# mmorise/World

Hardware: AMD Instinct MI355X
Metric: analysis frames/sec (Harvest+CheapTrick+D4C, 48 kHz, 5 ms hop) (higher is better)
Workload: dtype f64; 1 GPU; configs[1]: 1 x (48 kHz, 10 s) utterance(s) per step, Harvest+CheapTrick+D4C, fft_size=2048, frame_period=5 ms, inputs/outputs in HBM, 12 independent jobs in flight (one HIP stream + context each, a different utterance per job); utterances_per_gpu=1, jobs_in_flight=12, parallelism=single GPU, no collective

## Files before the change

world_amd/csrc/bandfilter.h:

```cpp
#pragma once
#include "trace.h"
#include "common.h"

namespace world_hip {

constexpr int kBpThreads = 256;
constexpr int kOutPer = 8;
constexpr int kTile = kBpThreads * kOutPer;
constexpr int kSegTiles = 2;
constexpr int kSeg = kTile * kSegTiles;
constexpr int kSegCap = kSeg / 2 + 2;

__host__ __device__ __forceinline__ int pad8(int i) { return i + (i >> 3); }

struct BandJob {
  const double *in;
  int in_len;
  int n;
  const double *taps;
  int ntap;
  int shift;
  int max_ntap;
  int nseg;
  double *seg_events;
// ... 147 lines not shown
    const int kbase = sub + tid * PER;
    unsigned mask[4] = {0u, 0u, 0u, 0u};
    {
      double a = kbase < len + 2 ? sample(kbase) : 0.0, b = kbase + 1 < len + 2 ? sample(kbase + 1) : 0.0;
#pragma unroll
      for (int q = 0; q < PER; ++q) {
        const double c = kbase + q + 2 < len + 2 ? sample(kbase + q + 2) : 0.0;
        const int i = t0 + kbase + q;
        const bool live = kbase + q < len;
        const double da = b - a, db = c - b;
        const bool r01 = live && i <= n - 2, r23 = live && i <= n - 3;
        if (r01 && 0.0 < a && b <= 0.0) mask[0] |= 1u << q;
        if (r01 && a < 0.0 && 0.0 <= b) mask[1] |= 1u << q;
        if (r23 && 0.0 < da && db <= 0.0) mask[2] |= 1u << q;
        if (r23 && da < 0.0 && 0.0 <= db) mask[3] |= 1u << q;
        a = b; b = c;
      }
    }
    WH_ACC_END(0);
    WH_ACC_BEGIN;
    unsigned long long packed = 0;
#pragma unroll
    for (int fam = 0; fam < 4; ++fam) packed |= (unsigned long long)__builtin_popcount(mask[fam]) << (16 * fam);
    unsigned long long total, off = block_excl_scan_u64<PRE>(packed, &total, scratch);
    WH_ACC_END(1);
    WH_ACC_BEGIN;
    int at[4];
#pragma unroll
    for (int fam = 0; fam < 4; ++fam) at[fam] = count[fam] + (int)((off >> (16 * fam)) & 0xFFFF);
    while ((mask[0] | mask[1] | mask[2] | mask[3]) != 0u) {
#pragma unroll
      for (int fam = 0; fam < 4; ++fam) {
        if (mask[fam] != 0u) {
          const int q = __builtin_ctz(mask[fam]);
          mask[fam] &= mask[fam] - 1;
          double a = sample(kbase + q), b = sample(kbase + q + 1);
          if (fam >= 2) { const double c = sample(kbase + q + 2); a = b - a; b = c - b; }
          if (at[fam] < cap) ev[fam * fam_stride + at[fam]] = fine_edge_fast(t0 + kbase + q + 1, a, b);
          ++at[fam];
        }
      }
    }
#pragma unroll
    for (int fam = 0; fam < 4; ++fam) count[fam] += (int)((total >> (16 * fam)) & 0xFFFF);
    WH_ACC_END(2);
  }
  WH_ACC_FLUSH(32, tid == 0);
}

__device__ __forceinline__ void band_events_segment(const BandJob &job, int seg) {
  DYN_LDS(lds);
  const int tid = threadIdx.x, nt = blockDim.x;
  const int n = job.n;
  const int seg_begin = seg * kSeg;
  int *cnt_out = job.seg_count + seg;
  if (seg_begin >= n) {
    if (tid == 0) for (int fam = 0; fam < 4; ++fam) cnt_out[(size_t)fam * job.nseg] = 0;
    return;
  }
  const int seg_end = imin(n, seg_begin + kSeg);
  const bool trace_me = blockIdx.x == 5 && blockIdx.y == 20; (void)trace_me;
  WH_ACC_DECL;
  WH_ACC_BEGIN;
  double *taps = reinterpret_cast<double *>(lds);
  double *yt = taps + (job.max_ntap + 1);
  double *s = yt + pad8(kTile + 2 + job.max_ntap + 3 + 8) + 1;
  double *scratch = s + pad8(kTile + 4) + 1;
  for (int j = tid; j < job.ntap; j += nt) taps[j] = job.taps[j];

  double *ev = job.seg_events + (size_t)seg * kSegCap;
  const size_t fam_stride = (size_t)job.nseg * kSegCap;
  int count[4] = {0, 0, 0, 0};
  const bool pipelined = tile_fits_regs(job);
  TileRegs pre;
  if (pipelined) tile_fetch(job, seg_begin, pre);
  WH_ACC_END(0);
  for (int t0 = seg_begin; t0 < seg_end; t0 += kTile) {
    WH_ACC_BEGIN;
    if (pipelined) {
      __syncthreads();
      tile_commit(job, pre, yt);
      __syncthreads();
      if (t0 + kTile < seg_end) tile_fetch(job, t0 + kTile, pre);
      WH_ACC_END(1);
      WH_ACC_BEGIN;
      fir_compute(job, taps, yt, s);
    } else {
      fir_tile(job, taps, t0, yt, s);
    }
    if (job.quirk) {
      const double qc = job.quirk[0], qs = job.quirk[1], q0 = job.quirk[2], w = job.quirk[3];
      const int n0 = t0 + tid + job.quirk_delay;
      double sn, cs, sr, cr;
      sincospi(n0 * w, &sn, &cs);
      sincospi(nt * w, &sr, &cr);
      const double sign = (n0 & 1) ? -1.0 : 1.0;
      for (int k = tid, j = 0; k < kTile + 2; k += nt, ++j) {
        const double flip = ((nt & 1) && (j & 1)) ? -sign : sign;
        s[pad8(k)] += flip * (qc * cs + qs * sn + q0);
        const double c2 = cs * cr - sn * sr;
        sn = sn * cr + cs * sr;
        cs = c2;
      }
      __syncthreads();
    }
    WH_ACC_END(2);
    WH_ACC_BEGIN;
    tile_events([&](int k) { return s[pad8(k)]; }, t0, kTile, n, ev, fam_stride, count, kSegCap, scratch);
    WH_ACC_END(3);
  }
  WH_ACC_SET(4, job.ntap);
  WH_ACC_FLUSH(16, tid == 0);
  if (tid == 0)
    for (int fam = 0; fam < 4; ++fam) cnt_out[(size_t)fam * job.nseg] = imin(count[fam], kSegCap);
}

inline size_t compact_lds_bytes(int nseg) { return 64 * sizeof(double) + sizeof(int) * (size_t)(nseg + 1); }
__device__ __forceinline__ void compact_event_segments(const double *seg_events, const int *seg_count, int nseg, int seg_cap,
                                                       double *events, int ev_cap, int *ev_count, char *lds) {
  double *scratch = reinterpret_cast<double *>(lds);
  int *pre = reinterpret_cast<int *>(scratch + 64);
  const int tid = threadIdx.x, nt = blockDim.x;
  int running = 0;
  for (int s0 = 0; s0 < nseg; s0 += nt) {
    const int s = s0 + tid;
    const int c = s < nseg ? seg_count[s] : 0;
    int tot;
    const int at = block_excl_scan_int(c, &tot, scratch);
    if (s < nseg) pre[s] = running + at;
    running += tot;
  }
  if (tid == 0) pre[nseg] = running;
  __syncthreads();
  const int total = imin(running, ev_cap);
  constexpr int kB = 8;
  int s = 0;
  for (int j0 = tid; j0 < total; j0 += kB * nt) {
    double v[kB];
#pragma unroll
    for (int q = 0; q < kB; ++q) {
      const int j = imin(j0 + q * nt, total - 1);
      while (j >= pre[s + 1]) ++s;
      v[q] = seg_events[(size_t)s * seg_cap + (j - pre[s])];
    }
#pragma unroll
    for (int q = 0; q < kB; ++q) if (j0 + q * nt < total) events[j0 + q * nt] = v[q];
  }
  if (tid == 0) *ev_count = total;
}

__device__ __forceinline__ double interval_loc(const double *e, int k, double fs) { return (e[k] + e[k + 1]) / 2.0 / fs; }
__device__ __forceinline__ double interval_f0(const double *e, int k, double fs) { return fs / (e[k + 1] - e[k]); }

__device__ __forceinline__ int intervals_at_or_before(const double *e, int n_int, double fs, double t) {
  int lo = 0, hi = n_int;
  if (n_int > 8) {
    const double first = interval_loc(e, 0, fs), last = interval_loc(e, n_int - 1, fs);
    const double r = (t - first) / (last - first) * (n_int - 1);
    int g = r < 0.0 ? 0 : (r > n_int - 1.0 ? n_int - 1 : static_cast<int>(r));
    if (interval_loc(e, g, fs) <= t) {
      lo = g + 1;
      for (int step = 1, q = g + 1; ; q += step, step <<= 1) {
        if (q >= n_int) break;
        if (interval_loc(e, q, fs) > t) { hi = q; break; }
        lo = q + 1;
      }
    } else {
      hi = g;
      for (int step = 1, q = g - 1; ; q -= step, step <<= 1) {
        if (q < 0) break;
        if (interval_loc(e, q, fs) <= t) { lo = q + 1; break; }
        hi = q;
      }
    }
  }
  while (lo < hi) {
    int mid = (lo + hi) >> 1;
    if (interval_loc(e, mid, fs) <= t) lo = mid + 1; else hi = mid;
  }
  return lo;
}

__device__ __forceinline__ int intervals_at_or_before_group(const double *e, int n_int, double fs, double t, int group, int sub) {
#ifdef WORLD_EMU
  (void)group; (void)sub;
  return intervals_at_or_before(e, n_int, fs, t);
#else
  if (n_int <= 0) return 0;
  const double first = interval_loc(e, 0, fs), last = interval_loc(e, n_int - 1, fs);
  if (!(first <= t)) return 0;
  if (last <= t) return n_int;
  int lo = 0, hi = n_int - 1;
  auto ones_at = [&](int idx, bool valid) {
    const bool pred = valid && interval_loc(e, idx, fs) <= t;
    return __popc((unsigned)(__ballot(pred) >> (32 * group)));
  };
  if (hi - lo > 32) {
    const double r = (t - first) / (last - first) * (n_int - 1);
    const int g = r < 0.0 ? 0 : (r > n_int - 1.0 ? n_int - 1 : static_cast<int>(r));
    int base = g - 15;
    base = base < lo + 1 ? lo + 1 : base;
    base = base > hi - 32 ? hi - 32 : base;
    const int ones = ones_at(base + sub, true);
    if (ones == 0) hi = base;
    else if (ones == 32) lo = base + 31;
    else return base + ones;
  }
  while (hi - lo > 32) {
    const int stride = (hi - lo + 31) / 32;
    const int idx = lo + (sub + 1) * stride;
    const int ones = ones_at(idx, idx < hi);
    const int nlo = lo + ones * stride, nhi = lo + (ones + 1) * stride;
    lo = nlo;
    hi = nhi < hi ? nhi : hi;
  }
  return lo + 1 + ones_at(lo + 1 + sub, lo + 1 + sub < hi);
#endif
}

__device__ __forceinline__ double interp_intervals(const double *e, int n_int, double fs, double t) {
  const int lo = intervals_at_or_before(e, n_int, fs, t);
  int k = lo < 1 ? 1 : (lo > n_int - 1 ? n_int - 1 : lo);
  double x0 = interval_loc(e, k - 1, fs), x1 = interval_loc(e, k, fs);
  double y0 = interval_f0(e, k - 1, fs), y1 = interval_f0(e, k, fs);
  double sl = (t - x0) / (x1 - x0);
  return y0 + sl * (y1 - y0);
}

struct IntervalRange {
  int c_first, c_last;
  int j_lo, m;
};
#ifndef HV_INTERVAL_CAP
#define HV_INTERVAL_CAP 288
#endif
constexpr int kIntervalCap = HV_INTERVAL_CAP;

__device__ __forceinline__ void interval_range_ends(const double *e, int n_int, double fs, double t, bool last,
                                                    IntervalRange *r) {
  const int c = intervals_at_or_before(e, n_int, fs, t);
  if (last) r->c_last = c; else r->c_first = c;
}
__device__ __forceinline__ void interval_range_close(int n_int, IntervalRange *r) {
  const int k_first = r->c_first < 1 ? 1 : (r->c_first > n_int - 1 ? n_int - 1 : r->c_first);
  const int k_last = r->c_last < 1 ? 1 : (r->c_last > n_int - 1 ? n_int - 1 : r->c_last);
  r->j_lo = k_first - 1;
  r->m = k_last - r->j_lo + 1;
}
__device__ __forceinline__ double interp_staged(const IntervalRange &r, const double *loc, const double *f0,
                                                int n_int, double t) {
  int lo = r.c_first, hi = r.c_last;
  while (lo < hi) {
    const int mid = (lo + hi) >> 1;
    if (loc[mid - r.j_lo] <= t) lo = mid + 1; else hi = mid;
  }
  const int k = (lo < 1 ? 1 : (lo > n_int - 1 ? n_int - 1 : lo)) - r.j_lo;
  const double x0 = loc[k - 1], x1 = loc[k], y0 = f0[k - 1], y1 = f0[k];
  const double sl = (t - x0) / (x1 - x0);
  return y0 + sl * (y1 - y0);
}

}
```

world_amd/csrc/harvest.hip:

```cpp
#ifndef HV_PLAIN_TID
#define WH_FRESH_TID
#endif
#include "bandfilter.h"
#include "decimate.h"
#include "harvest.h"
#include "trace.h"
WH_TRACE_DEFINE(hv)

namespace world_hip {

__global__ void __launch_bounds__(kDecThreads) hv_decimate_fwd(HarvestParams p, IirCoef c) {
  DYN_LDS(lds);
  const int u = blockIdx.y;
  dec_forward_block(p.b.x + (size_t)u * p.b.x_stride, p.b.x_len[u], p.lag, c, blockIdx.x,
                    p.fwd + (size_t)u * p.m_stride, reinterpret_cast<double *>(lds), dec_warm(p.ratio));
}
__global__ void __launch_bounds__(kDecThreads) hv_decimate_bwd(HarvestParams p, IirCoef c) {
  DYN_LDS(lds);
  const int u = blockIdx.y;
  dec_backward_block(p.fwd + (size_t)u * p.m_stride, p.b.x_len[u], p.lag, p.ratio, c, blockIdx.x,
                     p.lag / p.ratio, p.y_len[u], p.y + (size_t)u * p.y_stride, reinterpret_cast<double *>(lds),
                     dec_warm(p.ratio), p.mean_part + (size_t)u * p.mean_parts);
}
__global__ void hv_copy_signal(HarvestParams p) {
// ... 105 lines not shown
}

__global__ void __launch_bounds__(256) hv_block_spectra(HarvestParams p) {
  DYN_LDS(lds);
  const int blk = blockIdx.x, u = blockIdx.y, n = p.y_len[u];
  if (blk >= p.nblk) {
    band_quirk_constants(p, blk - p.nblk, u, reinterpret_cast<double *>(lds));
    return;
  }
  const int m0 = blk * p.fft_seg - p.fft_pre;
  if (blk * p.fft_seg >= n) return;
  cplx *Z = reinterpret_cast<cplx *>(lds);
  const TwLds tw = stage_twiddles(reinterpret_cast<double *>(lds) + kBandFft, kBandFftLg - 1, p.tab.tw);
  const double *y = p.y + (size_t)u * p.y_stride;
  for (int i = threadIdx.x; i < kBandFft; i += blockDim.x) {
    const int idx = m0 + i;
    rfft_in(Z, i) = (idx >= 0 && idx < n) ? y[idx] : 0.0;
  }
  double2 *out = p.blk_spec + ((size_t)u * p.nblk + blk) * kBandFftBins;
#ifdef WORLD_EMU
  block_rfft<3>(Z, kBandFftLg, tw, [&](int k, double re, double im) { out[k] = make_double2(re, im); });
#else
  {
    constexpr FftPlan plan = make_plan_max(kBandFftLg - 1, 3);
    block_cfft_dif_static<kBandFftLg - 1, 3, 256>(Z, tw);
    rfft_merge_items<(kBandFft / 4 + 1 + 255) / 256, 256>(Z, kBandFftLg, plan, tw,
      [&](int, int k, double ar, double ai, bool paired, double br, double bi) {
        out[k] = make_double2(ar, ai);
        if (paired) out[kBandFft / 2 - k] = make_double2(br, bi);
      });
  }
#endif
}

#ifndef HV_FFT_MIN_WAVES
#define HV_FFT_MIN_WAVES 4
#endif
template <bool REC>
__global__ void __launch_bounds__(kBandFftThreads, HV_FFT_MIN_WAVES) hv_band_events_fft(HarvestParams p) {
  DYN_LDS(lds);
  const int band = blockIdx.x, chunk = blockIdx.y, ue = blockIdx.z, u = ue + p.ev_u0, tid = threadIdx.x, nt = blockDim.x;
  const int n = p.y_len[u];
  const size_t list = ((size_t)(ue * p.nch + band) * 4);
  int *cnt_out = p.seg_count + list * p.nseg + chunk;
  const int blk0 = chunk * p.chunk_blocks;
  if (blk0 * p.fft_seg >= n) {
    if (tid == 0) for (int fam = 0; fam < 4; ++fam) cnt_out[(size_t)fam * p.nseg] = 0;
    return;
  }
  const int blk1 = imin(blk0 + p.chunk_blocks, (n + p.fft_seg - 1) / p.fft_seg);
  const bool trace_me = blockIdx.x == 20 && blockIdx.y == 0 && u == WH_TRACE_UTT; (void)trace_me;
  WH_STAMP(24, 0);
  cplx *Z = reinterpret_cast<cplx *>(lds);
  double *scratch = reinterpret_cast<double *>(lds) + kBandFft;
  const TwLds tw = stage_twiddles(scratch + 64, kBandFftLg - 1, p.tab.tw);
  WH_STAMP(24, 1);
  const double2 *H = p.band_spec + (size_t)band * kBandFftBins;
  const int shift = p.band_half[band] + 1;
  const int at0 = p.fft_pre + shift;
  const double *qc4 = p.quirk + ((size_t)u * p.nch + band) * kQuirkDoubles;
  const double qc = qc4[0], qs = qc4[1], q0 = qc4[2], w = qc4[3];
  double *ev = p.seg_events + (list * p.nseg + chunk) * p.seg_cap;
  const size_t fam_stride = (size_t)p.nseg * p.seg_cap;
  int count[4] = {0, 0, 0, 0};
#ifdef WORLD_EMU
  for (int blk = blk0; blk < blk1; ++blk) {
    const int t0 = blk * p.fft_seg;
    const double2 *X = p.blk_spec + ((size_t)u * p.nblk + blk) * kBandFftBins;
    auto product = [&](int k) { const double2 x = X[k], h = H[k]; cplx a, b; a.re = x.x; a.im = x.y; b.re = h.x; b.im = h.y; return cmul(a, b); };
    block_irfft<3>(Z, kBandFftLg, tw, product);
    const int len = imin(p.fft_seg, n - t0);
    for (int k = tid; k < len + 2; k += nt) {
      const int ng = t0 + k + shift;
      double sn, cs;
      sincospi(ng * w, &sn, &cs);
      rfft_in(Z, k + at0) += ((ng & 1) ? -1.0 : 1.0) * (qc * cs + qs * sn + q0);
    }
    tile_events<16, false>([&](int k) { return rfft_in(Z, k + at0); }, t0, len, n, ev, fam_stride, count, p.seg_cap, scratch);
  }
#else
  double sr, cr, sb, cb, sn0, cs0;
  if constexpr (!REC) {
    sincospi(nt * w, &sr, &cr);
    sincospi(p.fft_seg * w, &sb, &cb);
  } else {
    sr = qc4[4]; cr = qc4[5]; sb = qc4[6]; cb = qc4[7];
  }
  sincospi((blk0 * p.fft_seg + tid + shift) * w, &sn0, &cs0);
  constexpr int NT = 256, kItems = (kBandFft / 4 + 1 + NT - 1) / NT;
  constexpr int hh = kBandFft / 2, qq = hh / 2;
  constexpr FftPlan plan = make_plan_max(kBandFftLg - 1, 3);
  cplx hk[kItems], hm[kItems];
#pragma unroll
  for (int m = 0; m < kItems; ++m) {
    const int k = tid + m * NT;
    hk[m].re = hk[m].im = hm[m].re = hm[m].im = 0.0;
    if (k <= qq) {
      const double2 a = H[k], b = H[hh - k];
      hk[m].re = a.x; hk[m].im = a.y; hm[m].re = b.x; hm[m].im = b.y;
    }
  }
  const cplx wbf = twiddle(tw, tid, kBandFftLg, -1);
  WH_STAMP(24, 2);
  for (int blk = blk0; blk < blk1; ++blk) {
    const int t0 = blk * p.fft_seg;
    const double2 *X = p.blk_spec + ((size_t)u * p.nblk + blk) * kBandFftBins;
    irfft_pretwiddle_items_w<kItems, NT>(Z, kBandFftLg, plan, [&](int m, int k, cplx &x, cplx &y, cplx &wk) {
      const double2 a = X[k], b = X[hh - k];
      cplx ca, cb2; ca.re = a.x; ca.im = a.y; cb2.re = b.x; cb2.im = b.y;
      x = cmul(ca, hk[m]); y = cmul(cb2, hm[m]);
      wk = cconj(mul_w16_fwd(wbf, m));
    });
    if (blk == blk0) WH_STAMP(24, 3);
    block_cfft_dit_static<kBandFftLg - 1, 3, NT>(Z, tw);
    if (blk == blk0) WH_STAMP(24, 4);
    const int len = imin(p.fft_seg, n - t0);
    {
      const int n0 = t0 + tid + shift;
      double sn = sn0, cs = cs0;
      { const double c2 = cs0 * cb - sn0 * sb; sn0 = sn0 * cb + cs0 * sb; cs0 = c2; }
      const double sign = (n0 & 1) ? -1.0 : 1.0;
      for (int k = tid, j = 0; k < len + 2; k += nt, ++j) {
        const double flip = ((nt & 1) && (j & 1)) ? -sign : sign;
        rfft_in(Z, k + at0) += flip * (qc * cs + qs * sn + q0);
        const double c2 = cs * cr - sn * sr;
        sn = sn * cr + cs * sr;
        cs = c2;
      }
      __syncthreads();
    }
    if (blk == blk0) WH_STAMP(24, 5);
    tile_events<16, false>([&](int k) { return rfft_in(Z, k + at0); }, t0, len, n, ev, fam_stride, count, p.seg_cap, scratch,
                           trace_me && blk == blk0);
    if (blk == blk0) WH_STAMP(24, 6);
  }
#endif
  if (tid == 0)
    for (int fam = 0; fam < 4; ++fam) cnt_out[(size_t)fam * p.nseg] = imin(count[fam], p.seg_cap);
}

__global__ void hv_compact_events(HarvestParams p) {
  DYN_LDS(lds);
  const int bf = blockIdx.x, ue = blockIdx.y;
  const size_t list = (size_t)ue * p.nch * 4 + bf;
  compact_event_segments(p.seg_events + list * p.nseg * p.seg_cap, p.seg_count + list * p.nseg, p.nseg, p.seg_cap,
                         p.events + list * p.ev_cap, p.ev_cap, p.ev_count + list, lds);
}

constexpr int kRawFrames = 256;
#ifndef HV_RAW_RUN
#define HV_RAW_RUN 256
#endif
constexpr int kRawRun = HV_RAW_RUN;
__device__ __forceinline__ double hv_gate(const HarvestParams &p, int band, double v0, double v1, double v2, double v3) {
  double c = (v0 + v1 + v2 + v3) / 4.0;
  const double fb = p.band_f0[band];
  if (c > fb * 1.1 || c < fb * 0.9 || c > p.f0_ceil || c < p.f0_floor) c = 0.0;
  return c;
}
#ifndef HV_RAW_MIN_WG
#define HV_RAW_MIN_WG 8
#endif
__global__ void __launch_bounds__(kRawFrames, HV_RAW_MIN_WG) hv_raw_candidates(HarvestParams p) {
  DYN_LDS(lds);
  const int band = blockIdx.x, ue = blockIdx.z, u = ue + p.ev_u0, tid = threadIdx.x, nt = blockDim.x;
  if (band >= p.nch) return;
  const int f_begin = blockIdx.y * kRawRun, f_end = imin(f_begin + kRawRun, p.nfb[u]);
  if (f_begin >= f_end) return;
  const int *cnt = p.ev_count + (ue * p.nch + band) * 4;
  const double *ev = p.events + ((size_t)(ue * p.nch + band) * 4) * p.ev_cap;
  double *out = p.raw + ((size_t)u * p.nch + band) * p.fb_stride;
  int n_int[4];
  bool ok = true;
  for (int fam = 0; fam < 4; ++fam) {
    n_int[fam] = cnt[fam] >= 2 ? cnt[fam] - 1 : 0;
    if (n_int[fam] - 2 <= 0) ok = false;
  }
  if (!ok) {
    for (int f = f_begin + tid; f < f_end; f += nt) out[f] = 0.0;
    return;
  }
  double *loc = reinterpret_cast<double *>(lds);
  double *fz = loc + 4 * kIntervalCap;
  IntervalRange *range = reinterpret_cast<IntervalRange *>(fz + 4 * kIntervalCap);
#ifdef WORLD_EMU
  for (int job = tid; job < 8; job += nt) {
    const int fam = job >> 1;
    const bool last = job & 1;
    interval_range_ends(ev + (size_t)fam * p.ev_cap, n_int[fam], p.afs, (last ? f_end - 1 : f_begin) * 1 / 1000.0, last,
                        range + fam);
  }
#else
  {
    static_assert(kRawFrames == 8 * 32, "one 32-lane group per (family, end)");
    const int job = tid >> 5, fam = job >> 1, sub = tid & 31;
    const bool last = job & 1;
    const int c = intervals_at_or_before_group(ev + (size_t)fam * p.ev_cap, n_int[fam], p.afs,
                                               (last ? f_end - 1 : f_begin) * 1 / 1000.0, (tid >> 5) & 1, sub);
    if (sub == 0) { if (last) range[fam].c_last = c; else range[fam].c_first = c; }
  }
#endif
  __syncthreads();
  for (int fam = tid; fam < 4; fam += nt) interval_range_close(n_int[fam], range + fam);
  __syncthreads();
  const bool staged = range[0].m <= kIntervalCap && range[1].m <= kIntervalCap && range[2].m <= kIntervalCap &&
                      range[3].m <= kIntervalCap;
  if (!staged) {
    for (int f = f_begin + tid; f < f_end; f += nt) {
      const double t = f * 1 / 1000.0;
      out[f] = hv_gate(p, band, interp_intervals(ev, n_int[0], p.afs, t), interp_intervals(ev + p.ev_cap, n_int[1], p.afs, t),
                       interp_intervals(ev + 2 * (size_t)p.ev_cap, n_int[2], p.afs, t),
                       interp_intervals(ev + 3 * (size_t)p.ev_cap, n_int[3], p.afs, t));
    }
    return;
  }
  {
    const int m0 = range[0].m, m1 = m0 + range[1].m, m2 = m1 + range[2].m, m3 = m2 + range[3].m;
    for (int job = tid; job < m3; job += nt) {
      const int fam = (job >= m0) + (job >= m1) + (job >= m2);
      const int i = job - (fam == 0 ? 0 : fam == 1 ? m0 : fam == 2 ? m1 : m2);
      const double *e = ev + (size_t)fam * p.ev_cap + range[fam].j_lo;
      loc[fam * kIntervalCap + i] = interval_loc(e, i, p.afs);
      fz[fam * kIntervalCap + i] = interval_f0(e, i, p.afs);
    }
  }
  __syncthreads();
  for (int f = f_begin + tid; f < f_end; f += nt) {
    const double t = f * 1 / 1000.0;
    double v[4];
#pragma unroll
    for (int fam = 0; fam < 4; ++fam)
      v[fam] = interp_staged(range[fam], loc + fam * kIntervalCap, fz + fam * kIntervalCap, n_int[fam], t);
    out[f] = hv_gate(p, band, v[0], v[1], v[2], v[3]);
  }
}

__global__ void hv_detect(HarvestParams p) {
  const int frame = flat_thread_x(), u = blockIdx.y;
  if (frame >= p.nfb[u]) return;
  const double *raw = p.raw + (size_t)u * p.nch * p.fb_stride + frame;
  double *out = p.cand_a + ((size_t)u * p.fb_stride + frame) * p.maxc;
  int cnt = 0, st = 0, prev = 0;
  double run_sum = 0.0;
  constexpr int kBatch = 19;
  auto fetch = [&](double (&v)[kBatch], int j0) __attribute__((always_inline)) {
#pragma unroll
    for (int q = 0; q < kBatch; ++q) v[q] = raw[(size_t)imin(j0 + q, p.nch - 1) * p.fb_stride];
  };
  auto walk = [&](const double (&v)[kBatch], int j0) __attribute__((always_inline)) {
#pragma unroll
    for (int q = 0; q < kBatch; ++q) {
      const int j = j0 + q;
      if (j >= p.nch || j == 0) continue;
      const int cur = (j == p.nch - 1) ? 0 : (v[q] > 0 ? 1 : 0);
      if (cur - prev == 1) { st = j; run_sum = 0.0; }
      if (cur - prev == -1 && j - st >= 10 && cnt < p.maxc) out[cnt++] = run_sum / (j - st);
      if (cur) run_sum += v[q];
      prev = cur;
    }
  };
  double va[kBatch], vb[kBatch];
  fetch(va, 0);
  for (int j0 = 0; j0 < p.nch; j0 += 2 * kBatch) {
    fetch(vb, j0 + kBatch);
    walk(va, j0);
    if (j0 + kBatch >= p.nch) break;
    fetch(va, j0 + 2 * kBatch);
    walk(vb, j0 + kBatch);
  }
  const int zcap = imin(p.maxc, (p.nch + 10) / 11 + 1);
  for (int j = cnt; j < zcap; ++j) out[j] = 0.0;
  if (cnt > 0) atomicMax(p.nc + u, cnt);
}

__device__ __forceinline__ int floor_log2_int(int v) { return 31 - __builtin_clz((unsigned)v); }

__global__ void hv_refine_frames(HarvestParams p) {
  DYN_LDS(lds);
  const int frame = wave_item_x(), u = blockIdx.y;
  if (frame >= p.nfb[u]) return;
  const int lane = lane_id();
  const int cap = p.refine_cap;
  double *yc = reinterpret_cast<double *>(lds) + (size_t)wave_in_block() * 3 * cap;
  cplx *yw = reinterpret_cast<cplx *>(yc + cap);
  const int nfb = p.nfb[u], nc = p.nc[u];
  const double *src = p.cand_a + (size_t)u * p.fb_stride * p.maxc;
  double *dst_f0 = p.cand_b + ((size_t)u * p.fb_stride + frame) * p.maxc;
  double *dst_sc = p.score_b + ((size_t)u * p.fb_stride + frame) * p.maxc;
  const double *y = p.y + (size_t)u * p.y_stride;
  const int y_len = p.y_len[u];
  const double fs = p.afs, inv_fs = 1.0 / fs;
  const double pos = frame * 1 / 1000.0;

  const bool trace_me = frame == 5 * WH_TRACE_FRAME && u == WH_TRACE_UTT; (void)trace_me;
  WH_ACC_DECL;
  WH_ACC_BEGIN;
  const int origin = mround(pos * fs) - cap / 2;
  {
    constexpr int kB = 6;
    for (int k0 = lane; k0 < cap; k0 += kB * WAVE) {
      double v[kB];
#pragma unroll
      for (int q = 0; q < kB; ++q) v[q] = y[imax(0, imin(y_len - 1, origin + k0 + q * WAVE))];
#pragma unroll
      for (int q = 0; q < kB; ++q) if (k0 + q * WAVE < cap) yc[k0 + q * WAVE] = v[q];
    }
  }
  wave_sync();
  WH_ACC_END(0);

  constexpr int LH = WAVE >= 8 ? 8 : 1;
  constexpr int G = WAVE / LH;
  constexpr int PG = 8;
  constexpr int kIter = (6 + LH - 1) / LH;
  constexpr int kM = (7 + G - 1) / G;
  const int hl = lane / G, g = lane % G;
  int c_hw = -1, c_first = 0;
  int c_idx[kIter];
  double c_are[kIter], c_aim[kIter], c_dre[kIter], c_dim[kIter];
  for (int q = 0; q < kIter; ++q) c_idx[q] = -1;

  struct Cand { double f0c, bins; int hw, first, lgN, nh; };
  auto cand_of = [&](int j, int m) {
    Cand c;
    const int sf = m == 0 ? frame : (m <= 3 ? frame - m : frame + (m - 3));
    c.f0c = (m < 7 && sf >= 0 && sf < nfb) ? src[(size_t)sf * p.maxc + j] : 0.0;
    const double f = c.f0c > 0.0 ? c.f0c : 1.0;
    c.hw = static_cast<int>(1.5 * fs / f + 1.0);
    c.lgN = 2 + floor_log2_int(2 * c.hw + 1);
    const double base0 = static_cast<double>(-c.hw) * inv_fs;
    c.first = mround((pos + base0) * fs + 0.001);
    c.nh = imin(static_cast<int>(fs / 2.0 / f), 6);
    c.bins = f * (1 << c.lgN) / fs;
    return c;
  };

  for (int j = 0; j < nc; ++j) {
    double k_are[kM][kIter], k_aim[kM][kIter], k_dre[kM][kIter], k_dim[kM][kIter], k_f0[kM];
    int k_idx[kM][kIter], k_lgn[kM];
    for (int q = 0; q < kM; ++q) k_f0[q] = 0.0;
#ifndef WORLD_EMU
    const Cand mine = cand_of(j, lane < 7 ? lane : 7);
#endif
    for (int mi = 0; mi < 7; ++mi) {
      const int m = mi < 4 ? 3 - mi : mi;
#ifndef WORLD_EMU
      const double f0c = readlane_f64(mine.f0c, m);
      if (!(f0c > 0.0)) continue;
      const double bins = readlane_f64(mine.bins, m);
      const int hw = __builtin_amdgcn_readlane(mine.hw, m), lgN = __builtin_amdgcn_readlane(mine.lgN, m);
      const int first = __builtin_amdgcn_readlane(mine.first, m), nh = __builtin_amdgcn_readlane(mine.nh, m);
#else
      const Cand cm = cand_of(j, m);
      const double f0c = cm.f0c;
      if (!(f0c > 0.0)) continue;
      const double bins = cm.bins;
      const int hw = cm.hw, lgN = cm.lgN, first = cm.first, nh = cm.nh;
#endif
      const int blen = 2 * hw + 1;
      const int N = 1 << lgN;
      const bool same_window = hw == c_hw && first == c_first;
#ifdef HV_REFINE_ROTATE
      const bool table_window = false;
#else
      const bool table_window = p.win_full != nullptr;
#endif
      if (!same_window && table_window) {
        WH_ACC_BEGIN;
        const double2 *wf = p.win_full + (size_t)hw * hw;
        wave_sync();
        constexpr int kB = 3;
        for (int i0 = lane; i0 < blen; i0 += kB * WAVE) {
          double2 t[kB];
#pragma unroll
          for (int q = 0; q < kB; ++q) t[q] = wf[imin(blen - 1, i0 + q * WAVE)];
#pragma unroll
          for (int q = 0; q < kB; ++q) {
            const int i = i0 + q * WAVE;
            if (i < blen) {
              const double xv = yc[imax(0, imin(cap - 1, first + i - 1 - origin))];
              cplx pr; pr.re = xv * t[q].x; pr.im = xv * t[q].y;
              yw[i] = pr;
            }
          }
        }
// ... 319 lines not shown
        }
#else
        ph[h][0][pg] = are; ph[h][1][pg] = aim; ph[h][2][pg] = dre; ph[h][3][pg] = dim;
#endif
      }
      }
#ifdef WORLD_EMU
      for (int h = 0; h < kH; ++h)
        for (int hi = 0; hi < 8 / G; ++hi)
          if (h == g + G * hi)
            for (int k = 0; k < 4; ++k) {
              const double *v = ph[h][k];
              keep[hi][k] = ((v[0] + v[1]) + (v[2] + v[3])) + ((v[7] + v[6]) + (v[5] + v[4]));
            }
#endif
      double num = 0.0, den = 0.0, sc = 0.0;
      for (int hi = 0; hi < 8 / G; ++hi) {
        const int h = g + G * hi;
        if (h >= nh) continue;
        const double a_re = keep[hi][0], a_im = keep[hi][1], d_re = keep[hi][2], d_im = keep[hi][3];
        const double pwv = a_re * a_re + a_im * a_im;
        const double niv = a_re * d_im - a_im * d_re;
        const double inst = pwv == 0.0 ? 0.0 : static_cast<double>(mround(bins * (h + 1))) * fs / N + niv / pwv * fs / 2.0 / kPi;
        const double amp = sqrt(pwv);
        num += amp * inst;
        den += amp * (h + 1.0);
        sc += fabs((inst / (h + 1.0) - f0c) / f0c);
      }
#ifndef WORLD_EMU
      num = oct_sum(num); den = oct_sum(den); sc = oct_sum(sc);
#endif
      if (g == 0 && sh < 7 && tf >= 0 && tf < nfb) {
        double rf0 = num / (den + kTiny);
        double rsc = 1.0 / (sc / nh + kTiny);
        if (rf0 < p.f0_floor || rf0 > p.f0_ceil || rsc < 2.5) { rf0 = 0.0; rsc = 0.0; }
        put(tf, j + nc * slot_m(d), rf0, rsc);
      }
    };
    if constexpr (SL == 8) refine_shift(lane / G);
    else for (int sh = lane / G; sh < kS; sh += SL) refine_shift(sh);
  }
}

__device__ __forceinline__ double nearest_error(double ref, const double *c, int nc) {
  double dmin = 1e300;
  for (int i = 0; i < nc; ++i) {
    const double d = fabs(ref - c[i]);
    dmin = d < dmin ? d : dmin;
  }
  const double e = dmin / ref;
  return e > 1.0 ? 1.0 : e;
}
constexpr int kPruneFrames = 16;
__global__ void hv_prune(HarvestParams p) {
  DYN_LDS(lds);
  double *rows = reinterpret_cast<double *>(lds);
  const int u = blockIdx.y, f0 = blockIdx.x * kPruneFrames;
  const int nfb = p.nfb[u];
  if (f0 >= nfb) return;
  const int nslot = p.nc[u] * 7;
  const int nrows = imin(kPruneFrames + 2, nfb - f0 + 1);
  const int nt = blockDim.x;
  if (nslot == 0) {
    for (int r = threadIdx.x; r < imin(kPruneFrames, nfb - f0); r += nt) p.c0[(size_t)u * p.fb_stride + f0 + r] = 0.0;
    return;
  }
  {
    constexpr int kB = 8;
    const int n = nrows * nslot;
    for (int i0 = threadIdx.x; i0 < n; i0 += kB * nt) {
      double v[kB];
#pragma unroll
      for (int q = 0; q < kB; ++q) {
        const int i = imin(i0 + q * nt, n - 1);
        const int r = i / nslot, j = i - r * nslot, f = imax(0, imin(nfb - 1, f0 - 1 + r));
        v[q] = p.cand_b[((size_t)u * p.fb_stride + f) * p.maxc + j];
      }
#pragma unroll
      for (int q = 0; q < kB; ++q) {
        const int i = i0 + q * nt;
        if (i < n) {
          const int f = f0 - 1 + i / nslot;
          rows[i] = (f >= 0 && f < nfb) ? v[q] : 0.0;
        }
      }
    }
  }
  __syncthreads();
  double *kept_sc = rows + (size_t)(kPruneFrames + 2) * nslot;
  {
    constexpr int kB = 4;
    const int n = imin(kPruneFrames, nfb - f0) * nslot;
    for (int i0 = threadIdx.x; i0 < n; i0 += kB * nt) {
      double scv[kB];
#pragma unroll
      for (int q = 0; q < kB; ++q) {
        const int i = imin(i0 + q * nt, n - 1);
        const int r = i / nslot, j = i - r * nslot;
        scv[q] = p.score_b[((size_t)u * p.fb_stride + f0 + r) * p.maxc + j];
      }
#pragma unroll
      for (int q = 0; q < kB; ++q) {
        const int i = i0 + q * nt;
        if (i >= n) break;
        const int r = i / nslot, j = i - r * nslot, frame = f0 + r;
        const size_t at = ((size_t)u * p.fb_stride + frame) * p.maxc + j;
        double ref = rows[(r + 1) * nslot + j], sc = scv[q];
        if (frame >= 1 && frame < nfb - 1 && ref != 0) {
          double e1 = nearest_error(ref, rows + (r + 2) * nslot, nslot);
          double e2 = nearest_error(ref, rows + r * nslot, nslot);
          if ((e1 < e2 ? e1 : e2) > 0.05) { ref = 0; sc = 0; }
        }
        p.cand_a[at] = ref;
        p.score_a[at] = sc;
        kept_sc[i] = sc;
      }
    }
  }
  __syncthreads();
  {
    const int lane = lane_id(), nfr = imin(kPruneFrames, nfb - f0);
    for (int r = wave_in_block(); r < nfr; r += waves_per_block()) {
      const double *c = rows + (size_t)(r + 1) * nslot, *sv = kept_sc + (size_t)r * nslot;
      double best = 0.0, top = 0.0;
      int slot = 0x7FFFFFFF;
      for (int j = lane; j < nslot; j += WAVE) {
        const double sj = sv[j];
        if (sj > top) { best = c[j]; top = sj; slot = j; }
      }
      const double wtop = wave_max(top);
      double v = 0.0;
      if (wtop > 0.0) {
        const int mine = top == wtop ? slot : 0x7FFFFFFF;
        const int win = -wave_max_int(-mine);
#ifndef WORLD_EMU
        v = readlane_f64(best, __builtin_amdgcn_readfirstlane(win % WAVE));
#else
        (void)win;
        v = best;
#endif
      }
      if (lane == 0) p.c0[(size_t)u * p.fb_stride + f0 + r] = v;
    }
  }
}

size_t hv_band_lds_bytes(int max_half) { return band_lds_bytes(2 * max_half + 1); }

void launch_harvest_raw(const HarvestParams &g, int G, int max_fb, int stages, hipStream_t stream) {
  if ((stages & 1) && !(g.fft_seg > 0 && g.nseg == 1))
    WH_BLOCKS(hv_compact_events, dim3(g.nch * 4, G), 256, compact_lds_bytes(g.nseg), stream, g);
  if (stages & 2)
    WH_BLOCKS(hv_raw_candidates, dim3((g.nch + 7) / 8 * 8, (max_fb + kRawRun - 1) / kRawRun, G), kRawFrames,
              8 * kIntervalCap * sizeof(double) + 4 * sizeof(IntervalRange), stream, g);
}
void launch_harvest_detect(const HarvestParams &p, int max_fb, hipStream_t stream) {
  WH_THREADS(hv_detect, max_fb, p.b.n_utt, 1, stream, p);
}

size_t hv_refine_lds_bytes(const HarvestParams &p) {
  return p.win_full && !p.refine_frames ? sizeof(double) * (3 * p.refine_cap + 6 * static_cast<int>(p.afs / 1000.0) + 2)
                                        : 3 * sizeof(double) * p.refine_cap;
}
void launch_harvest_refine(const HarvestParams &p, int max_fb, hipStream_t stream) {
  if (p.win_full && !p.refine_frames) WH_WAVES(hv_refine, max_fb, p.b.n_utt, 1, hv_refine_lds_bytes(p), stream, p);
  else WH_WAVES(hv_refine_frames, max_fb, p.b.n_utt, 1, hv_refine_lds_bytes(p), stream, p);
}

void launch_harvest(const HarvestParams &p, int max_x_len, int max_y_len, int max_fb, int max_frames,
                    hipStream_t stream) {
  const int B = p.b.n_utt;
  if (p.ratio == 1) {
    WH_THREADS(hv_copy_signal, max_y_len, B, 1, stream, p);
  } else {
    IirCoef c = decimate_coef(p.ratio);
    const int spans = (max_x_len + 2 * p.lag + 2 * kDecPad + kDecSpan - 1) / kDecSpan;
    WH_BLOCKS(hv_decimate_fwd, dim3(spans, B), kDecThreads, dec_lds_bytes(), stream, p, c);
    WH_BLOCKS(hv_decimate_bwd, dim3(spans, B), kDecThreads, dec_lds_bytes(), stream, p, c);
  }
  if (p.ratio == 1) WH_BLOCKS(hv_partial_sums, dim3(p.mean_parts, B), 256, 64 * sizeof(double), stream, p);
  WH_BLOCKS(hv_remove_mean, dim3(p.nyq_slices, B), 256, 64 * sizeof(double), stream, p);
  const size_t lds = sizeof(double) * (kBandFft + 64 + twiddle_lds_doubles(kBandFftLg - 1));
  if (p.fft_seg > 0) WH_BLOCKS(hv_block_spectra, dim3(p.nblk + p.nch, B), 256, lds, stream, p);
  else WH_BLOCKS(hv_band_quirk, dim3(p.nch, B), 64, 64 * sizeof(double), stream, p);
  for (int u0 = 0; u0 < B; u0 += p.ev_group) {
    HarvestParams g = p;
    g.ev_u0 = u0;
    const int G = imin(p.ev_group, B - u0);
    if (p.fft_seg > 0 && p.inkernel_consts)
      devrt::launch_blocks("hv_band_events_fft", hv_band_events_fft<false>, dim3(p.nch, p.nseg, G), kBandFftThreads, lds, stream, g);
    else if (p.fft_seg > 0)
      devrt::launch_blocks("hv_band_events_fft", hv_band_events_fft<true>, dim3(p.nch, p.nseg, G), kBandFftThreads, lds, stream, g);
    else WH_BLOCKS(hv_band_events, dim3(p.nseg, p.nch, G), kBpThreads, hv_band_lds_bytes(p.max_half), stream, g);
    launch_harvest_raw(g, G, max_fb, 3, stream);
  }
  launch_harvest_detect(p, max_fb, stream);
  launch_harvest_refine(p, max_fb, stream);
  launch_harvest_tail(p, max_fb, max_frames, stream);
}

void launch_harvest_tail(const HarvestParams &p, int max_fb, int max_frames, hipStream_t stream) {
  const int B = p.b.n_utt;
  WH_BLOCKS(hv_prune, dim3((max_fb + kPruneFrames - 1) / kPruneFrames, B), 256,
            sizeof(double) * (size_t)(2 * kPruneFrames + 2) * p.maxc, stream, p);
  launch_harvest_contour(p, max_fb, max_frames, stream);
}

}
```

Measured before the change: 4.431 million frames/s.

## Replace per-frame binary search with scatter-count-scan of interval crossings in raw candidates

In hv_raw_candidates, each staged interval location is now mapped to the first frame at or after it. The kernel atomically tallies these per-frame counts into packed 16-bit LDS counters, and a block-wide exclusive scan then gives every frame its interval index for all four families. This replaces the per-frame, per-family binary search over staged locations. Separately, the interval searches compare against a margin-scaled t*fs, avoiding the divisions when the result is unambiguous, and the initial guess uses float math. In exchange the kernel adds LDS atomics, an extra scan and sync, reuses the fz buffer as scratch, and adds careful rounding-boundary handling.

After: 4.395 million frames/s. No clear change (-0.8%).

```diff
diff --git a/world_amd/csrc/bandfilter.h b/world_amd/csrc/bandfilter.h
--- a/world_amd/csrc/bandfilter.h
+++ b/world_amd/csrc/bandfilter.h
@@ -323,31 +323,58 @@
 __device__ __forceinline__ double interval_loc(const double *e, int k, double fs) { return (e[k] + e[k + 1]) / 2.0 / fs; }
 __device__ __forceinline__ double interval_f0(const double *e, int k, double fs) { return fs / (e[k + 1] - e[k]); }
 
+struct LocAtOrBefore {
+  double t, fs, T, below, above;
+  __device__ __forceinline__ LocAtOrBefore(double t_, double fs_) : t(t_), fs(fs_), T(t_ * fs_) {
+    below = T * (1.0 - 0x1p-50);
+    above = T * (1.0 + 0x1p-50);
+    const bool margins = t > 0.0 && fs > 0.0 && __builtin_isnormal(t) && __builtin_isnormal(fs) && __builtin_isnormal(T) &&
+                         __builtin_isnormal(below) && __builtin_isnormal(above);
+    if (!margins) below = above = __builtin_nan("");
+  }
+  __device__ __forceinline__ int cheap(const double *e, int k) const {
+    const double h = (e[k] + e[k + 1]) * 0.5;
+    if (__builtin_isnormal(h)) {
+      if (h <= below) return 1;
+      if (h >= above) return 0;
+    }
+    return -1;
+  }
+  __device__ __forceinline__ bool operator()(const double *e, int k) const {
+    const int c = cheap(e, k);
+    return c >= 0 ? c != 0 : interval_loc(e, k, fs) <= t;
+  }
+  __device__ __forceinline__ int guess(const double *e, int n_int) const {
+    const double hf = (e[0] + e[1]) * 0.5, hl = (e[n_int - 1] + e[n_int]) * 0.5;
+    const float r = static_cast<float>(T - hf) / static_cast<float>(hl - hf) * static_cast<float>(n_int - 1);
+    return r > 0.0f ? (r < static_cast<float>(n_int - 1) ? static_cast<int>(r) : n_int - 1) : 0;
+  }
+};
+
 __device__ __forceinline__ int intervals_at_or_before(const double *e, int n_int, double fs, double t) {
+  const LocAtOrBefore at(t, fs);
   int lo = 0, hi = n_int;
   if (n_int > 8) {
-    const double first = interval_loc(e, 0, fs), last = interval_loc(e, n_int - 1, fs);
-    const double r = (t - first) / (last - first) * (n_int - 1);
-    int g = r < 0.0 ? 0 : (r > n_int - 1.0 ? n_int - 1 : static_cast<int>(r));
-    if (interval_loc(e, g, fs) <= t) {
+    const int g = at.guess(e, n_int);
+    if (at(e, g)) {
       lo = g + 1;
       for (int step = 1, q = g + 1; ; q += step, step <<= 1) {
         if (q >= n_int) break;
-        if (interval_loc(e, q, fs) > t) { hi = q; break; }
+        if (!at(e, q)) { hi = q; break; }
         lo = q + 1;
       }
     } else {
       hi = g;
       for (int step = 1, q = g - 1; ; q -= step, step <<= 1) {
         if (q < 0) break;
-        if (interval_loc(e, q, fs) <= t) { lo = q + 1; break; }
+        if (at(e, q)) { lo = q + 1; break; }
         hi = q;
       }
     }
   }
   while (lo < hi) {
     int mid = (lo + hi) >> 1;
-    if (interval_loc(e, mid, fs) <= t) lo = mid + 1; else hi = mid;
+    if (at(e, mid)) lo = mid + 1; else hi = mid;
   }
   return lo;
 }
@@ -358,17 +385,16 @@
   return intervals_at_or_before(e, n_int, fs, t);
 #else
   if (n_int <= 0) return 0;
-  const double first = interval_loc(e, 0, fs), last = interval_loc(e, n_int - 1, fs);
-  if (!(first <= t)) return 0;
-  if (last <= t) return n_int;
+  const LocAtOrBefore at(t, fs);
+  if (!at(e, 0)) return 0;
+  if (at(e, n_int - 1)) return n_int;
   int lo = 0, hi = n_int - 1;
   auto ones_at = [&](int idx, bool valid) {
-    const bool pred = valid && interval_loc(e, idx, fs) <= t;
+    const bool pred = valid && at(e, idx);
     return __popc((unsigned)(__ballot(pred) >> (32 * group)));
   };
   if (hi - lo > 32) {
-    const double r = (t - first) / (last - first) * (n_int - 1);
-    const int g = r < 0.0 ? 0 : (r > n_int - 1.0 ? n_int - 1 : static_cast<int>(r));
+    const int g = at.guess(e, n_int);
     int base = g - 15;
     base = base < lo + 1 ? lo + 1 : base;
     base = base > hi - 32 ? hi - 32 : base;
@@ -418,17 +444,34 @@
   r->j_lo = k_first - 1;
   r->m = k_last - r->j_lo + 1;
 }
-__device__ __forceinline__ double interp_staged(const IntervalRange &r, const double *loc, const double *f0,
-                                                int n_int, double t) {
-  int lo = r.c_first, hi = r.c_last;
-  while (lo < hi) {
-    const int mid = (lo + hi) >> 1;
-    if (loc[mid - r.j_lo] <= t) lo = mid + 1; else hi = mid;
-  }
-  const int k = (lo < 1 ? 1 : (lo > n_int - 1 ? n_int - 1 : lo)) - r.j_lo;
+__device__ __forceinline__ double interp_staged(int count, int j_lo, const double *loc, const double *f0, int n_int, double t) {
+  const int k = (count < 1 ? 1 : (count > n_int - 1 ? n_int - 1 : count)) - j_lo;
   const double x0 = loc[k - 1], x1 = loc[k], y0 = f0[k - 1], y1 = f0[k];
   const double sl = (t - x0) / (x1 - x0);
   return y0 + sl * (y1 - y0);
 }
 
-}
+__device__ __forceinline__ double frame_time_1ms(int g) { return g * 1 / 1000.0; }
+
+__device__ __forceinline__ int first_frame_at_or_after(double loc, int lo, int hi) {
+  const double x = loc * 1000.0;
+  if (!(x < hi + 2.0)) return hi + 1;
+  if (x <= lo - 1.0) return lo;
+  int g = static_cast<int>(ceil(x));
+  if (!(x <= g * (1.0 - 0x1p-50) && x >= (g - 1) * (1.0 + 0x1p-50))) {
+    int c = g - 1;
+    while (c <= g && !(loc <= frame_time_1ms(c))) ++c;
+    g = c;
+  }
+  return g < lo ? lo : (g > hi ? hi + 1 : g);
+}
+
+__device__ __forceinline__ void lds_add_u64(unsigned long long *p, unsigned long long v) {
+#ifdef WORLD_EMU
+  *p += v;
+#else
+  atomicAdd(p, v);
+#endif
+}
+
+}
diff --git a/world_amd/csrc/harvest.hip b/world_amd/csrc/harvest.hip
--- a/world_amd/csrc/harvest.hip
+++ b/world_amd/csrc/harvest.hip
@@ -281,6 +281,16 @@
 #define HV_RAW_RUN 256
 #endif
 constexpr int kRawRun = HV_RAW_RUN;
+constexpr int kRawStageJobs = (4 * kIntervalCap + kRawFrames - 1) / kRawFrames;
+constexpr int kRawScanWords = 8;
+#ifdef WORLD_EMU
+constexpr size_t kRawLdsBytes = 8 * kIntervalCap * sizeof(double) + 4 * sizeof(IntervalRange) + kRawRun * sizeof(unsigned long long);
+#else
+constexpr size_t kRawLdsBytes = 8 * kIntervalCap * sizeof(double) + 4 * sizeof(IntervalRange);
+static_assert(kRawRun + kRawScanWords <= 4 * kIntervalCap, "the counters and the scan's scratch lie over fz");
+static_assert(kRawFrames / 64 <= kRawScanWords, "a scratch word per wavefront");
+#endif
+static_assert(kIntervalCap <= 65535, "a family's staged intervals fit a 16-bit field of a frame's counter, summed over the run too");
 __device__ __forceinline__ double hv_gate(const HarvestParams &p, int band, double v0, double v1, double v2, double v3) {
   double c = (v0 + v1 + v2 + v3) / 4.0;
   const double fb = p.band_f0[band];
@@ -313,6 +323,13 @@
   double *fz = loc + 4 * kIntervalCap;
   IntervalRange *range = reinterpret_cast<IntervalRange *>(fz + 4 * kIntervalCap);
 #ifdef WORLD_EMU
+  unsigned long long *tally = reinterpret_cast<unsigned long long *>(range + 4);
+#else
+  unsigned long long *tally = reinterpret_cast<unsigned long long *>(fz);
+  unsigned long long counts1 = 0;
+#endif
+  for (int i = tid; i < kRawRun; i += nt) tally[i] = 0;
+#ifdef WORLD_EMU
   for (int job = tid; job < 8; job += nt) {
     const int fam = job >> 1;
     const bool last = job & 1;
@@ -345,21 +362,64 @@
   }
   {
     const int m0 = range[0].m, m1 = m0 + range[1].m, m2 = m1 + range[2].m, m3 = m2 + range[3].m;
-    for (int job = tid; job < m3; job += nt) {
+    auto stage = [&](int job, int *slot) __attribute__((always_inline)) {
       const int fam = (job >= m0) + (job >= m1) + (job >= m2);
       const int i = job - (fam == 0 ? 0 : fam == 1 ? m0 : fam == 2 ? m1 : m2);
-      const double *e = ev + (size_t)fam * p.ev_cap + range[fam].j_lo;
-      loc[fam * kIntervalCap + i] = interval_loc(e, i, p.afs);
-      fz[fam * kIntervalCap + i] = interval_f0(e, i, p.afs);
-    }
-  }
+      const int j_lo = range[fam].j_lo, at = j_lo + i;
+      const double *e = ev + (size_t)fam * p.ev_cap + j_lo;
+      const double l = interval_loc(e, i, p.afs);
+      *slot = fam * kIntervalCap + i;
+      loc[*slot] = l;
+      if (at >= range[fam].c_first && at < range[fam].c_last) {
+        const int g = first_frame_at_or_after(l, f_begin + 1, f_end - 1);
+        if (g < f_end) lds_add_u64(tally + (g - f_begin), 1ull << (16 * fam));
+      }
+      return interval_f0(e, i, p.afs);
+    };
+#ifdef WORLD_EMU
+    for (int job = tid; job < m3; job += nt) {
+      int slot;
+      const double y = stage(job, &slot);
+      fz[slot] = y;
+    }
+  }
+#else
+    double fzr[kRawStageJobs];
+    int slot[kRawStageJobs];
+#pragma unroll
+    for (int q = 0; q < kRawStageJobs; ++q)
+      if (tid + q * kRawFrames < m3) fzr[q] = stage(tid + q * kRawFrames, &slot[q]);
+    __syncthreads();
+    static_assert(kRawRun <= kRawFrames, "one frame per thread: the scan leaves a frame's counts with its thread");
+    const int f1 = f_begin + tid;
+    const unsigned long long mine = f1 < f_end ? tally[tid] : 0;
+    unsigned long long total;
+    counts1 = block_excl_scan_u64<false>(mine, &total, reinterpret_cast<double *>(tally + kRawRun)) + mine;
+    __syncthreads();
+#pragma unroll
+    for (int q = 0; q < kRawStageJobs; ++q)
+      if (tid + q * kRawFrames < m3) fz[slot[q]] = fzr[q];
+  }
+#endif
   __syncthreads();
+  int c_first[4], j_lo[4];
+#pragma unroll
+  for (int fam = 0; fam < 4; ++fam) { c_first[fam] = range[fam].c_first; j_lo[fam] = range[fam].j_lo; }
+#ifdef WORLD_EMU
+  unsigned long long counts = 0;
+#endif
   for (int f = f_begin + tid; f < f_end; f += nt) {
-    const double t = f * 1 / 1000.0;
+#ifdef WORLD_EMU
+    counts += tally[f - f_begin];
+#else
+    const unsigned long long counts = counts1;
+#endif
+    const double t = frame_time_1ms(f);
     double v[4];
 #pragma unroll
     for (int fam = 0; fam < 4; ++fam)
-      v[fam] = interp_staged(range[fam], loc + fam * kIntervalCap, fz + fam * kIntervalCap, n_int[fam], t);
+      v[fam] = interp_staged(c_first[fam] + static_cast<int>((counts >> (16 * fam)) & 0xffffu), j_lo[fam], loc + fam * kIntervalCap,
+                             fz + fam * kIntervalCap, n_int[fam], t);
     out[f] = hv_gate(p, band, v[0], v[1], v[2], v[3]);
   }
 }
@@ -985,7 +1045,7 @@
     WH_BLOCKS(hv_compact_events, dim3(g.nch * 4, G), 256, compact_lds_bytes(g.nseg), stream, g);
   if (stages & 2)
     WH_BLOCKS(hv_raw_candidates, dim3((g.nch + 7) / 8 * 8, (max_fb + kRawRun - 1) / kRawRun, G), kRawFrames,
-              8 * kIntervalCap * sizeof(double) + 4 * sizeof(IntervalRange), stream, g);
+              kRawLdsBytes, stream, g);
 }
 void launch_harvest_detect(const HarvestParams &p, int max_fb, hipStream_t stream) {
   WH_THREADS(hv_detect, max_fb, p.b.n_utt, 1, stream, p);
```
